# PyLops/pylops-mpi

Measured on AMD Instinct MI355X. Metric: MPIFirstDerivative fp64 matvec+rmatvec pairs/sec, higher is better.
Workload: dtype f64; 1 GPU; MPIFirstDerivative cgls config (BASELINE configs[1]); partition=scatter-axis0, kind=centered, order=3

## Files before the change

include/pam.h:

```cpp
#ifndef PAM_H
#define PAM_H

#include <stdint.h>

#ifdef __cplusplus
extern "C" {
#endif

#define PAM_F64 0
#define PAM_F32 1
#define PAM_C128 2
#define PAM_C64 3

#define PAM_EARG   (-1)
#define PAM_EDTYPE (-2)
#define PAM_EOP    (-3)

int64_t pam_version(void);

int64_t pam_reduce_ws_elems(void);

int pam_fill(void* stream, void* y, int64_t n, double value, int dtype);
int pam_neg(void* stream, void* y, const void* x, int64_t n, int dtype);
int pam_add(void* stream, void* y, const void* a, const void* b, int64_t n,
            int dtype);
int pam_sub(void* stream, void* y, const void* a, const void* b, int64_t n,
            int dtype);
int pam_mul(void* stream, void* y, const void* a, const void* b, int64_t n,
            int dtype);
int pam_scale(void* stream, void* y, const void* x, double alpha, int64_t n,
              int dtype);
int pam_axpy(void* stream, void* y, const void* x, double alpha, int64_t n,
             int dtype);
int pam_xpby(void* stream, void* y, const void* x, double beta, int64_t n,
             int dtype);

int pam_axpy_d(void* stream, void* y, const void* x, const void* alpha,
               double scale, int64_t n, int dtype);
int pam_xpby_d(void* stream, void* y, const void* x, const void* beta,
               double scale, int64_t n, int dtype);
int pam_scalar_alpha(void* stream, void* out, const void* num,
                     const void* den, double damp);
int pam_scalar_div(void* stream, void* out, const void* num, const void* den);

int pam_cmul(void* stream, void* y, const void* a, const void* b, int64_t n,
             int dtype);
int pam_cscale(void* stream, void* y, const void* x, double alpha_re,
               double alpha_im, int64_t n, int dtype);
int pam_conj(void* stream, void* y, const void* x, int64_t n, int dtype);

int pam_thresh(void* stream, void* y, const void* x, int64_t n, int kind,
               double thresh, int dtype);

int pam_dot(void* stream, const void* x, const void* y, int64_t n, void* ws,
            void* out, int dtype);

int pam_cdot(void* stream, const void* x, const void* y, int64_t n,
             int conjx, void* ws, void* out, int dtype);

int pam_norm_local(void* stream, const void* x, int64_t n, int op, double p,
                   void* ws, void* out, int dtype);

#define PAM_GROUP_MAX 4
int pam_group_shrink(void* stream, int mode, int64_t ncomp,
                     void* y0, void* y1, void* y2, void* y3,
                     const void* a0, const void* a1, const void* a2,
                     const void* a3,
                     const void* b0, const void* b1, const void* b2,
                     const void* b3,
                     double beta, int64_t n, double thresh, int dtype);
int pam_group_norm(void* stream, int64_t ncomp,
                   const void* x0, const void* x1, const void* x2,
                   const void* x3,
                   int64_t n, void* ws, void* out, int dtype);

int64_t pam_fd_halo_width(int op);
int pam_fd_apply(void* stream, int op, int edge, const void* x,
                 const void* gf, const void* gb, void* y, int64_t nloc,
                 int64_t m, int64_t row0, int64_t nglob, int64_t rbegin,
                 int64_t rend, double coeff, int dtype);

int pam_nsconv(void* stream, int forward, const void* x, void* y,
               const void* hs, int64_t batch, int64_t d, int64_t m,
               int64_t nf, int64_t hsize, double oh, double dh, int dtype);

int pam_fd_serial(void* stream, int op, int edge, const void* x, void* y,
                  int64_t batch, int64_t d, int64_t m, double coeff,
                  int dtype);

int64_t pam_gemv_ws_elems(int64_t nr, int64_t nc);
int pam_gemv(void* stream, int trans, const void* A, const void* x, void* y,
             int64_t nr, int64_t nc, void* ws, int dtype);

int pam_gemm(void* stream, const void* A, const void* B, void* C, int64_t M,
             int64_t N, int64_t K, int64_t lda, int64_t ldb, int64_t ldc,
             int accumulate, int dtype);
int pam_transpose(void* stream, const void* A, void* At, int64_t nr,
                  int64_t nc, int dtype);

int pam_cgemm_batched(void* stream, const void* A, const void* B, void* C,
                      int64_t batch, int64_t M, int64_t N, int64_t K,
                      int64_t strideA, int64_t strideB, int64_t strideC,
                      int opa, int accumulate, int dtype);

int pam_gemm_batched(void* stream, const void* A, const void* B, void* C,
                     int64_t batch, int64_t M, int64_t N, int64_t K,
                     int64_t strideA, int64_t strideB, int64_t strideC,
                     int opa, int accumulate, int dtype);

int pam_unzip(void* stream, void* dst_real, const void* src_cplx, int64_t n,
              int dtype);
int pam_zip(void* stream, void* dst_cplx, const void* src_real, int64_t n,
            int dtype);

int pam_rfft_strided(void* stream, const void* in_real, void* out_cplx,
                     int64_t nt, int64_t m, int dtype);
int pam_irfft_strided(void* stream, void* in_cplx, void* out_real,
                      int64_t nt, int64_t m, int dtype);

int pam_rfft_contig(void* stream, const void* in_real, void* out_cplx,
                    int64_t nt, int64_t m, int dtype);
int pam_irfft_contig(void* stream, void* in_cplx, void* out_real,
                     int64_t nt, int64_t m, int dtype);

int pam_unzip_t(void* stream, void* dst_real, const void* src_cplx,
                int64_t nt, int64_t m, int dtype);
int pam_zip_t(void* stream, void* dst_cplx, const void* src_real,
              int64_t nt, int64_t m, int dtype);

int pam_gemm_kt(void* stream, const void* At, const void* B, void* C,
                int64_t M, int64_t N, int64_t K, int accumulate,
                int dtype);

int pam_ctranspose(void* stream, const void* A, void* At, int64_t nr,
                   int64_t nc, int conj, int dtype);

#ifdef __cplusplus
}
#endif
#endif
```

pylops_mpi_amd/_ffi.py:

```python
import ctypes
import os

import torch

_LIB_PATH = os.path.join(os.path.dirname(os.path.abspath(__file__)),
                         "libpam.so")
_lib = None
_load_error = None

F64, F32, C128, C64 = 0, 1, 2, 3
_CODES = {torch.float64: F64, torch.float32: F32,
          torch.complex128: C128, torch.complex64: C64}

P, L, I, D = (ctypes.c_void_p, ctypes.c_int64, ctypes.c_int,
              ctypes.c_double)
_SIGS = {
    "pam_version": ([], L),
    "pam_reduce_ws_elems": ([], L),
    "pam_fill": ([P, P, L, D, I], I),
    "pam_neg": ([P, P, P, L, I], I),
    "pam_add": ([P, P, P, P, L, I], I),
    "pam_sub": ([P, P, P, P, L, I], I),
    "pam_mul": ([P, P, P, P, L, I], I),
    "pam_scale": ([P, P, P, D, L, I], I),
    "pam_axpy": ([P, P, P, D, L, I], I),
    "pam_xpby": ([P, P, P, D, L, I], I),
    "pam_axpy_d": ([P, P, P, P, D, L, I], I),
    "pam_xpby_d": ([P, P, P, P, D, L, I], I),
    "pam_scalar_alpha": ([P, P, P, P, D], I),
    "pam_scalar_div": ([P, P, P, P], I),
    "pam_dot": ([P, P, P, L, P, P, I], I),
    "pam_cmul": ([P, P, P, P, L, I], I),
    "pam_cscale": ([P, P, P, D, D, L, I], I),
    "pam_conj": ([P, P, P, L, I], I),
    "pam_thresh": ([P, P, P, L, I, D, I], I),
    "pam_cdot": ([P, P, P, L, I, P, P, I], I),
    "pam_cgemm_batched": ([P, P, P, P, L, L, L, L, L, L, L, I, I, I], I),
    "pam_ctranspose": ([P, P, P, L, L, I, I], I),
    "pam_rfft_strided": ([P, P, P, L, L, I], I),
    "pam_irfft_strided": ([P, P, P, L, L, I], I),
    "pam_rfft_contig": ([P, P, P, L, L, I], I),
    "pam_irfft_contig": ([P, P, P, L, L, I], I),
    "pam_unzip_t": ([P, P, P, L, L, I], I),
    "pam_zip_t": ([P, P, P, L, L, I], I),
    "pam_unzip": ([P, P, P, L, I], I),
    "pam_zip": ([P, P, P, L, I], I),
    "pam_gemm_batched": ([P, P, P, P, L, L, L, L, L, L, L, I, I, I], I),
    "pam_norm_local": ([P, P, L, I, D, P, P, I], I),
    "pam_group_shrink": ([P, I, L, P, P, P, P, P, P, P, P, P, P, P, P, D, L,
                          D, I], I),
    "pam_group_norm": ([P, L, P, P, P, P, L, P, P, I], I),
    "pam_gemv_ws_elems": ([L, L], L),
    "pam_gemv": ([P, I, P, P, P, L, L, P, I], I),
    "pam_gemm": ([P, P, P, P, L, L, L, L, L, L, I, I], I),
    "pam_gemm_kt": ([P, P, P, P, L, L, L, I, I], I),
    "pam_transpose": ([P, P, P, L, L, I], I),
    "pam_fd_halo_width": ([I], L),
    "pam_nsconv": ([P, I, P, P, P, L, L, L, L, L, D, D, I], I),
    "pam_fd_serial": ([P, I, I, P, P, L, L, L, D, I], I),
    "pam_fd_apply": ([P, I, I, P, P, P, P, L, L, L, L, L, L, D, I], I),
}


def lib():
    global _lib, _load_error
    if _lib is not None:
        return _lib
    if _load_error is not None:
        raise _load_error
    try:
        so = ctypes.CDLL(_LIB_PATH)
        for name, (argtypes, restype) in _SIGS.items():
            fn = getattr(so, name)
            fn.argtypes = argtypes
            fn.restype = restype
        ver = so.pam_version()
        if ver != 1:
            raise RuntimeError(f"pam ABI version mismatch: {ver}")
    except OSError as e:
        _load_error = ImportError(
            f"pam HIP extension not found/loadable at {_LIB_PATH} "
            f"(build it with __graft_entry__.build()): {e}")
        raise _load_error
    _lib = so
    return so


def available() -> bool:
    try:
        lib()
        return True
    except ImportError:
        return False


def checked(rc: int, what: str) -> None:
    if rc != 0:
        raise RuntimeError(f"pam: {what} failed with code {rc}")


def dtype_code(torch_dtype) -> int:
    try:
        return _CODES[torch_dtype]
    except KeyError:
        raise TypeError(f"pam: unsupported dtype {torch_dtype}") from None
```

pylops_mpi_amd/csrc/pam.hip:

```cpp

#include <hip/hip_runtime.h>
#include <math.h>
#include <stdint.h>
#include <stdlib.h>
#include <utility>

#include "../../include/pam.h"
#include "fd_defs.h"

#define PAM_ABI_VERSION 1
#define BLK 256
#define NPARTIAL 1024

extern "C" int64_t pam_version(void) { return PAM_ABI_VERSION; }
extern "C" int64_t pam_reduce_ws_elems(void) { return NPARTIAL; }

static inline int check(hipError_t e) { return (int)e; }

static inline int64_t grid_1d(int64_t work) {
  static int64_t cap = [] {
    const char* e = getenv("PAM_EW_CAP");
    return (int64_t)(e ? atoll(e) : 0x7FFFFFFF);
  }();
  int64_t g = (work + BLK - 1) / BLK;
// ... 957 lines not shown
static int group_norm_nc(void* stream, int64_t ncomp, const void* const* x,
                         int64_t n, void* ws, void* out) {
  switch (ncomp) {
    case 1: return group_norm_launch<T, CPLX, 1>(stream, x, n, ws, out);
    case 2: return group_norm_launch<T, CPLX, 2>(stream, x, n, ws, out);
    case 3: return group_norm_launch<T, CPLX, 3>(stream, x, n, ws, out);
    default: return group_norm_launch<T, CPLX, 4>(stream, x, n, ws, out);
  }
}

extern "C" int pam_group_norm(void* stream, int64_t ncomp, const void* x0,
                              const void* x1, const void* x2, const void* x3,
                              int64_t n, void* ws, void* out, int dtype) {
  const void* const x[PAM_GROUP_MAX] = {x0, x1, x2, x3};
  if (ncomp < 1 || ncomp > PAM_GROUP_MAX) return PAM_EARG;
  for (int64_t c = 0; c < ncomp; ++c)
    if (!x[c]) return PAM_EARG;
  if (n < 0 || !ws || !out) return PAM_EARG;
  if (dtype < PAM_F64 || dtype > PAM_C64) return PAM_EDTYPE;
  if (n == 0)
    return check(hipMemsetAsync(out, 0, sizeof(double), (hipStream_t)stream));
  switch (dtype) {
    case PAM_F64: return group_norm_nc<double, false>(stream, ncomp, x, n, ws, out);
    case PAM_F32: return group_norm_nc<float, false>(stream, ncomp, x, n, ws, out);
    case PAM_C128: return group_norm_nc<double, true>(stream, ncomp, x, n, ws, out);
    default: return group_norm_nc<float, true>(stream, ncomp, x, n, ws, out);
  }
}

#define GEMV_CHUNKS 64

extern "C" int64_t pam_gemv_ws_elems(int64_t nr, int64_t nc) {
  (void)nr;
  return GEMV_CHUNKS * nc;
}

template <typename T, int V>
__global__ void __launch_bounds__(BLK) gemv_n_kernel(
    const T* __restrict__ A, const T* __restrict__ x, T* __restrict__ y,
    int64_t nr, int64_t nc) {
  const int64_t wave = ((int64_t)blockIdx.x * (BLK / 64))
                       + (threadIdx.x >> 6);
  const int lane = threadIdx.x & 63;
  const int64_t nwaves = (int64_t)gridDim.x * (BLK / 64);
  const int64_t ncv = nc / V;
  for (int64_t r = wave; r < nr; r += nwaves) {
    const T* __restrict__ row = A + r * nc;
    double acc = 0.0;
    for (int64_t cv = lane; cv < ncv; cv += 64) {
      T a[V], b[V];
      loadv<T, V>(row + cv * V, a);
      loadv<T, V>(x + cv * V, b);
#pragma unroll
      for (int k = 0; k < V; ++k) acc += (double)a[k] * (double)b[k];
    }
    for (int64_t c = ncv * V + lane; c < nc; c += 64)
      acc += (double)row[c] * (double)x[c];
#pragma unroll
    for (int off = 32; off > 0; off >>= 1) acc += __shfl_down(acc, off, 64);
    if (lane == 0) y[r] = (T)acc;
  }
}

template <typename T, int V>
__global__ void __launch_bounds__(BLK) gemv_t_stage1(
    const T* __restrict__ A, const T* __restrict__ x,
    double* __restrict__ partials, int64_t nr, int64_t nc) {
  const int64_t c0 = ((int64_t)blockIdx.x * BLK + threadIdx.x) * V;
  const int chunk = blockIdx.y;
  const int64_t r0 = (nr * chunk) / GEMV_CHUNKS;
  const int64_t r1 = (nr * (chunk + 1)) / GEMV_CHUNKS;
  if (c0 >= nc) return;
  double acc[V] = {};
  for (int64_t r = r0; r < r1; ++r) {
    T v[V];
    loadv<T, V>(A + r * nc + c0, v);
#pragma unroll
    for (int j = 0; j < V; ++j)
      acc[j] += (double)v[j] * (double)x[r];
  }
#pragma unroll
  for (int j = 0; j < V; ++j)
    partials[(int64_t)chunk * nc + c0 + j] = acc[j];
}

template <typename T>
__global__ void __launch_bounds__(BLK) gemv_t_stage2(
    const double* __restrict__ partials, T* __restrict__ y, int64_t nc) {
  const int64_t c = (int64_t)blockIdx.x * BLK + threadIdx.x;
  if (c >= nc) return;
  double acc = 0.0;
  for (int ch = 0; ch < GEMV_CHUNKS; ++ch)
    acc += partials[(int64_t)ch * nc + c];
  y[c] = (T)acc;
}

template <typename T>
static int gemv_launch(void* stream, int trans, const void* A, const void* x,
                       void* y, int64_t nr, int64_t nc, void* ws) {
  if (nr <= 0 || nc <= 0 || !A || !x || !y) return PAM_EARG;
  hipStream_t s = (hipStream_t)stream;
  if (!trans) {
    constexpr int V = VecW<T>::value;
    const bool vec_ok = (nc % V == 0) && ((uintptr_t)A % 16 == 0) &&
                        ((uintptr_t)x % 16 == 0);
    int64_t nb = (nr + (BLK / 64) - 1) / (BLK / 64);
    if (nb > 4096) nb = 4096;
    if (vec_ok)
      hipLaunchKernelGGL((gemv_n_kernel<T, V>), dim3((uint32_t)nb), dim3(BLK),
                         0, s, (const T*)A, (const T*)x, (T*)y, nr, nc);
    else
      hipLaunchKernelGGL((gemv_n_kernel<T, 1>), dim3((uint32_t)nb), dim3(BLK),
                         0, s, (const T*)A, (const T*)x, (T*)y, nr, nc);
    return check(hipGetLastError());
  }
  if (!ws) return PAM_EARG;
  constexpr int V = VecW<T>::value;
  const bool vec_ok = (nc % V == 0) && ((uintptr_t)A % 16 == 0);
  const int64_t ncl = vec_ok ? nc / V : nc;
  dim3 g1((uint32_t)((ncl + BLK - 1) / BLK), GEMV_CHUNKS);
  if (vec_ok)
    hipLaunchKernelGGL((gemv_t_stage1<T, V>), g1, dim3(BLK), 0, s,
                       (const T*)A, (const T*)x, (double*)ws, nr, nc);
  else
    hipLaunchKernelGGL((gemv_t_stage1<T, 1>), g1, dim3(BLK), 0, s,
                       (const T*)A, (const T*)x, (double*)ws, nr, nc);
  hipError_t e = hipGetLastError();
  if (e != hipSuccess) return (int)e;
  hipLaunchKernelGGL((gemv_t_stage2<T>),
                     dim3((uint32_t)((nc + BLK - 1) / BLK)), dim3(BLK), 0, s,
                     (const double*)ws, (T*)y, nc);
  return check(hipGetLastError());
}

extern "C" int pam_gemv(void* stream, int trans, const void* A, const void* x,
                        void* y, int64_t nr, int64_t nc, void* ws, int dtype) {
  if (dtype == PAM_F64)
    return gemv_launch<double>(stream, trans, A, x, y, nr, nc, ws);
  if (dtype == PAM_F32)
    return gemv_launch<float>(stream, trans, A, x, y, nr, nc, ws);
  return PAM_EDTYPE;
}


extern "C" int64_t pam_fd_halo_width(int op) {
  switch (op) {
    case 0: case 1: case 2: case 3: case 4: case 5: return 1;
    case 6: case 7: case 8: case 9: case 10: case 11: case 12: case 13:
      return 2;
    default: return PAM_EOP;
  }
}

template <typename T, int OP, int V, bool NTS = false, bool RSWAP = false>
__global__ void __launch_bounds__(BLK) fd_kernel(Rows<T> R, T* __restrict__ y,
                                                 int64_t row0, int64_t N, T c,
                                                 int edge, int64_t rbegin,
                                                 int64_t rend) {
  const int64_t brow = RSWAP ? blockIdx.x : blockIdx.y;
  const int64_t grows = RSWAP ? gridDim.x : gridDim.y;
  const int64_t bcol = RSWAP ? blockIdx.y : blockIdx.x;
  const int64_t gcols = RSWAP ? gridDim.y : gridDim.x;
  const int64_t m = R.m, mv = m / V;
  const int64_t cstride = (int64_t)gcols * blockDim.x;
  for (int64_t i = rbegin + brow; i < rend; i += grows) {
    const int64_t g = row0 + i;
    T* __restrict__ yrow = y + i * m;
    for (int64_t jv = (int64_t)bcol * blockDim.x + threadIdx.x; jv < mv;
         jv += cstride) {
      const int64_t j = jv * V;
      T acc[V];
#pragma unroll
      for (int k = 0; k < V; ++k) acc[k] = (T)0;
#pragma unroll
      for (int t = 0; t < FDDef<OP>::NT; ++t) {
        const Term tm = FDDef<OP>::TERMS[t];
        if (g >= tm.lo && g <= N - 1 - tm.hi) {
          T v[V];
          loadv<T, V>(R.row(i + tm.off) + j, v);
#pragma unroll
          for (int k = 0; k < V; ++k) acc[k] += (T)tm.coeff * v[k];
        }
      }
      if (edge) fd_edge<T, OP, V>(R, i, j, g, N, acc);
#pragma unroll
      for (int k = 0; k < V; ++k) acc[k] *= c;
      storev_p<T, V, NTS>(yrow + j, acc);
    }
    if constexpr (V > 1) {
      for (int64_t j = mv * V + (int64_t)bcol * blockDim.x + threadIdx.x;
           j < m; j += cstride) {
        T acc[1] = {(T)0};
#pragma unroll
        for (int t = 0; t < FDDef<OP>::NT; ++t) {
          const Term tm = FDDef<OP>::TERMS[t];
          if (g >= tm.lo && g <= N - 1 - tm.hi)
            acc[0] += (T)tm.coeff * R.row(i + tm.off)[j];
        }
        if (edge) fd_edge<T, OP, 1>(R, i, j, g, N, acc);
        const T o = acc[0] * c;
        if constexpr (NTS)
          __builtin_nontemporal_store(o, yrow + j);
        else
          yrow[j] = o;
      }
    }
  }
}


template <typename T, int OP, int V, int W, int t>
__device__ __forceinline__ void roll_term(const T (&win)[2 * W + 1][V],
                                          T (&acc)[V], int64_t g,
                                          int64_t N) {
  constexpr Term tm = FDDef<OP>::TERMS[t];
  if (g >= tm.lo && g <= N - 1 - tm.hi) {
#pragma unroll
    for (int k = 0; k < V; ++k)
      acc[k] += (T)tm.coeff * win[tm.off + W][k];
  }
}

template <typename T, int OP, int V, int W, int... Ts>
__device__ __forceinline__ void roll_terms(const T (&win)[2 * W + 1][V],
                                           T (&acc)[V], int64_t g,
                                           int64_t N,
                                           std::integer_sequence<int, Ts...>) {
  (roll_term<T, OP, V, W, Ts>(win, acc, g, N), ...);
}

template <typename T, int OP, int V, int CV, bool NTS = false,
          bool NTL = false>
__global__ void __launch_bounds__(BLK) fd_roll_kernel(
    Rows<T> R, T* __restrict__ y, int64_t row0, int64_t N, T c, int edge,
    int64_t rbegin, int64_t rend) {
  constexpr int W = FDDef<OP>::W;
  constexpr int NROLL = 2 * W + 1;
  const int64_t m = R.m, mv = m / V;
  const int64_t base = (int64_t)blockIdx.x * blockDim.x * CV + threadIdx.x;
  const int64_t nr = rend - rbegin;
  const int64_t c0 = rbegin + (nr * blockIdx.y) / gridDim.y;
  const int64_t c1 = rbegin + (nr * (blockIdx.y + 1)) / gridDim.y;
  if (c1 <= c0 || base >= mv) return;
  const int64_t lo = R.gf ? -(int64_t)R.w : 0;
  const int64_t hi = R.nloc - 1 + (R.gb ? R.w : 0);
  auto clamp_row = [&](int64_t i) {
    return i < lo ? lo : (i > hi ? hi : i);
  };
  int64_t js[CV];
  bool vq[CV];
#pragma unroll
  for (int q = 0; q < CV; ++q) {
    const int64_t jq = base + (int64_t)q * blockDim.x;
    vq[q] = jq < mv;
    js[q] = (vq[q] ? jq : mv - 1) * V;
  }
  T buf[CV][NROLL][V];
#pragma unroll
  for (int q = 0; q < CV; ++q)
#pragma unroll
    for (int k = 0; k < NROLL; ++k)
      if constexpr (NTL) loadv_nt<T, V>(R.row(clamp_row(c0 - W + k)) + js[q], buf[q][k]);
      else loadv<T, V>(R.row(clamp_row(c0 - W + k)) + js[q], buf[q][k]);
  for (int64_t i = c0; i < c1; ++i) {
    const int64_t g = row0 + i;
    T nxt[CV][V];
    const int64_t rn = clamp_row(i + 1 + W);
#pragma unroll
    for (int q = 0; q < CV; ++q)
      if constexpr (NTL) loadv_nt<T, V>(R.row(rn) + js[q], nxt[q]);
      else loadv<T, V>(R.row(rn) + js[q], nxt[q]);
#pragma unroll
    for (int q = 0; q < CV; ++q) {
      T acc[V];
#pragma unroll
      for (int k = 0; k < V; ++k) acc[k] = (T)0;
      roll_terms<T, OP, V, W>(
          buf[q], acc, g, N,
          std::make_integer_sequence<int, FDDef<OP>::NT>{});
      if (edge) fd_edge<T, OP, V>(R, i, js[q], g, N, acc);
#pragma unroll
      for (int k = 0; k < V; ++k) acc[k] *= c;
      if (vq[q]) storev_p<T, V, NTS>(y + i * m + js[q], acc);
#pragma unroll
      for (int k = 0; k < NROLL - 1; ++k)
#pragma unroll
        for (int v = 0; v < V; ++v) buf[q][k][v] = buf[q][k + 1][v];
#pragma unroll
      for (int v = 0; v < V; ++v) buf[q][NROLL - 1][v] = nxt[q][v];
    }
  }
}

template <int... Us, typename F>
__device__ __forceinline__ void fd_static_for(
    std::integer_sequence<int, Us...>, F&& f) {
  (f(std::integral_constant<int, Us>{}), ...);
}

template <typename T, int OP, int V, int W, int ROT, int t>
__device__ __forceinline__ void roll2_term(const T (&win)[2 * W + 1][V],
                                           T (&acc)[V], int64_t g,
                                           int64_t N) {
  constexpr Term tm = FDDef<OP>::TERMS[t];
  constexpr int NR = 2 * W + 1;
  constexpr int slot = ((tm.off + W + ROT) % NR + NR) % NR;
  if (g >= tm.lo && g <= N - 1 - tm.hi) {
#pragma unroll
    for (int k = 0; k < V; ++k)
      acc[k] += (T)tm.coeff * win[slot][k];
  }
}

template <typename T, int OP, int V, int W, int ROT, int... Ts>
__device__ __forceinline__ void roll2_terms(
    const T (&win)[2 * W + 1][V], T (&acc)[V], int64_t g, int64_t N,
    std::integer_sequence<int, Ts...>) {
  (roll2_term<T, OP, V, W, ROT, Ts>(win, acc, g, N), ...);
}

template <typename T, int OP, int V, int CV, bool NTS = false>
__global__ void __launch_bounds__(BLK) fd_roll2_kernel(
    Rows<T> R, T* __restrict__ y, int64_t row0, int64_t N, T c, int edge,
    int64_t rbegin, int64_t rend) {
  constexpr int W = FDDef<OP>::W;
  constexpr int NROLL = 2 * W + 1;
  const int64_t m = R.m, mv = m / V;
  const int64_t base = (int64_t)blockIdx.x * blockDim.x * CV + threadIdx.x;
  const int64_t nr = rend - rbegin;
  const int64_t c0 = rbegin + (nr * blockIdx.y) / gridDim.y;
  const int64_t c1 = rbegin + (nr * (blockIdx.y + 1)) / gridDim.y;
  if (c1 <= c0 || base >= mv) return;
  const int64_t lo = R.gf ? -(int64_t)R.w : 0;
  const int64_t hi = R.nloc - 1 + (R.gb ? R.w : 0);
  auto clamp_row = [&](int64_t i) {
    return i < lo ? lo : (i > hi ? hi : i);
  };
  int64_t js[CV];
  bool vq[CV];
#pragma unroll
  for (int q = 0; q < CV; ++q) {
    const int64_t jq = base + (int64_t)q * blockDim.x;
    vq[q] = jq < mv;
    js[q] = (vq[q] ? jq : mv - 1) * V;
  }
  T buf[CV][NROLL][V];
#pragma unroll
  for (int q = 0; q < CV; ++q)
#pragma unroll
    for (int k = 0; k < NROLL; ++k)
      loadv<T, V>(R.row(clamp_row(c0 - W + k)) + js[q], buf[q][k]);
  int64_t i = c0;
  auto step = [&](auto rotc) {
    constexpr int ROT = decltype(rotc)::value;
    constexpr int oldest = ROT % NROLL;
    const int64_t rn = clamp_row(i + W + 1);
    T nxt[CV][V];
#pragma unroll
    for (int q = 0; q < CV; ++q)
      loadv<T, V>(R.row(rn) + js[q], nxt[q]);
    const int64_t g = row0 + i;
#pragma unroll
    for (int q = 0; q < CV; ++q) {
      T acc[V];
#pragma unroll
      for (int k = 0; k < V; ++k) acc[k] = (T)0;
      roll2_terms<T, OP, V, W, ROT>(
          buf[q], acc, g, N,
          std::make_integer_sequence<int, FDDef<OP>::NT>{});
      if (edge) fd_edge<T, OP, V>(R, i, js[q], g, N, acc);
#pragma unroll
      for (int k = 0; k < V; ++k) acc[k] *= c;
      if (vq[q]) storev_p<T, V, NTS>(y + i * m + js[q], acc);
#pragma unroll
      for (int v = 0; v < V; ++v) buf[q][oldest][v] = nxt[q][v];
    }
    ++i;
  };
  while (i + NROLL <= c1)
    fd_static_for(std::make_integer_sequence<int, NROLL>{},
                  [&](auto rc) { step(rc); });
  fd_static_for(std::make_integer_sequence<int, NROLL>{}, [&](auto rc) {
    if (i < c1) step(rc);
  });
}

static int fd_vec_override() {
  static int v = [] {
    const char* e = getenv("PAM_FD_VEC");
    return e ? atoi(e) : 0;
  }();
  return v;
}

static int fd_nt_override() {
  static int v = [] {
    const char* e = getenv("PAM_FD_NT");
    return e ? atoi(e) : 0;
  }();
  return v;
}

template <typename T, int OP>
static int fd_launch(void* stream, int edge, const void* x, const void* gf,
                     const void* gb, void* y, int64_t nloc, int64_t m,
                     int64_t row0, int64_t nglob, int64_t rbegin,
                     int64_t rend, double coeff) {
  if (nloc < 0 || m <= 0 || rbegin < 0 || rend > nloc) return PAM_EARG;
  const int64_t nrows = rend - rbegin;
  if (nloc == 0 || nrows <= 0) return 0;
  Rows<T> R{(const T*)x, (const T*)gf, (const T*)gb, nloc, m, FDDef<OP>::W};
  const bool align16 = ((uintptr_t)x % 16 == 0) && ((uintptr_t)y % 16 == 0) &&
                       (gf == nullptr || (uintptr_t)gf % 16 == 0) &&
                       (gb == nullptr || (uintptr_t)gb % 16 == 0);
  int V = 1;
  if (align16) {
    if (sizeof(T) == 8)
      V = (m % 2 == 0) ? 2 : 1;
    else
      V = (m % 4 == 0) ? 4 : 1;
    const int ov = fd_vec_override();
    if ((ov == 1 || ov == 2 || ov == 4) && m % ov == 0) V = ov;
  }
  const int64_t mv = m / V;
  static int gycap = [] {
    const char* e = getenv("PAM_FD_GY");
    return e ? atoi(e) : 65535;
  }();
  static int totcap = [] {
    const char* e = getenv("PAM_FD_CAP");
    return e ? atoi(e) : 262144;
  }();
  int gy = (int)(nrows < gycap ? nrows : gycap);
  if (gy < 1) gy = 1;
  int64_t gx64 = (mv + BLK - 1) / BLK;
  int64_t cap = totcap / gy;
  if (cap < 1) cap = 1;
  if (gx64 > cap) gx64 = cap;
  dim3 grid((uint32_t)gx64, (uint32_t)gy);
  hipStream_t s = (hipStream_t)stream;
  static int rollov = [] {
    const char* e = getenv("PAM_FD_ROLL");
    return e ? atoi(e) : 0;
  }();
  static int64_t longrow = [] {
    const char* e = getenv("PAM_FD_LONGROW");
    return (int64_t)(e ? atoll(e) : (4 << 20));
  }();
  const int64_t rowbytes = m * (int64_t)sizeof(T);
  const bool roll_auto =
      rollov == 0 && V > 1 &&
      (rowbytes > longrow ||
       (rowbytes * 8 >= longrow * 5 && (nrows % 1024) != 0));
  static int rolltgt = [] {
    const char* e = getenv("PAM_FD_ROLL_TGT");
    return e ? atoi(e) : 2048;
  }();
  if ((rollov > 0 && V > 1) || roll_auto) {
    if (roll_auto && fd_vec_override() == 0 && m % 4 == 0 && align16)
      V = 4;
    static int cvov = [] {
      const char* e = getenv("PAM_FD_ROLL_CV");
      return e ? atoi(e) : 8;
    }();
    const int CV = (cvov == 2 || cvov == 4) ? cvov : 8;
    const int64_t mv2 = m / V;
    int64_t gx = (mv2 + (int64_t)BLK * CV - 1) / ((int64_t)BLK * CV);
    int64_t gyr = rolltgt / (gx ? gx : 1);
    const int64_t minchunk = 16;
    int64_t maxgy = (nrows + minchunk - 1) / minchunk;
    if (gyr > maxgy) gyr = maxgy;
    if (gyr < 1) gyr = 1;
    if (gyr > 65535) gyr = 65535;
    dim3 gridr((uint32_t)gx, (uint32_t)gyr);
    const bool rnt = fd_nt_override() != 0;
    static int ntlov = [] {
      const char* e = getenv("PAM_FD_NTL");
      return e ? atoi(e) : 0;
    }();
    const bool rntl = ntlov != 0;
#define ROLL_LAUNCH(KER, VV, CC)                                              \
  do {                                                                        \
    if (rnt)                                                                  \
      hipLaunchKernelGGL((KER<T, OP, VV, CC, true>), gridr, dim3(BLK), 0, s,  \
                         R, (T*)y, row0, nglob, (T)coeff, edge, rbegin,       \
                         rend);                                               \
    else                                                                      \
      hipLaunchKernelGGL((KER<T, OP, VV, CC, false>), gridr, dim3(BLK), 0, s, \
                         R, (T*)y, row0, nglob, (T)coeff, edge, rbegin,       \
                         rend);                                               \
  } while (0)
#define ROLL_LAUNCH1(VV, CC)                                                  \
  do {                                                                        \
    if (rntl)                                                                 \
      hipLaunchKernelGGL((fd_roll_kernel<T, OP, VV, CC, false, true>),        \
                         gridr, dim3(BLK), 0, s, R, (T*)y, row0, nglob,       \
                         (T)coeff, edge, rbegin, rend);                       \
    else                                                                      \
      ROLL_LAUNCH(fd_roll_kernel, VV, CC);                                    \
  } while (0)
    if (rollov == 2) {
      if (V == 4 && CV == 2) ROLL_LAUNCH(fd_roll2_kernel, 4, 2);
      else if (V == 4 && CV == 8) ROLL_LAUNCH(fd_roll2_kernel, 4, 8);
      else if (V == 4) ROLL_LAUNCH(fd_roll2_kernel, 4, 4);
      else if (CV == 2) ROLL_LAUNCH(fd_roll2_kernel, 2, 2);
      else if (CV == 8) ROLL_LAUNCH(fd_roll2_kernel, 2, 8);
      else ROLL_LAUNCH(fd_roll2_kernel, 2, 4);
    } else {
      if (V == 4 && CV == 2) ROLL_LAUNCH1(4, 2);
      else if (V == 4 && CV == 8) ROLL_LAUNCH1(4, 8);
      else if (V == 4) ROLL_LAUNCH1(4, 4);
      else if (CV == 2) ROLL_LAUNCH1(2, 2);
      else if (CV == 8) ROLL_LAUNCH1(2, 8);
      else ROLL_LAUNCH1(2, 4);
    }
#undef ROLL_LAUNCH1
#undef ROLL_LAUNCH
    return check(hipGetLastError());
  }
  static int rswap = [] {
    const char* e = getenv("PAM_FD_RSWAP");
    return e ? atoi(e) : 0;
  }();
  if (rswap) {
    dim3 grid_s((uint32_t)gy, (uint32_t)gx64);
    if (V == 4)
      hipLaunchKernelGGL((fd_kernel<T, OP, 4, false, true>), grid_s,
                         dim3(BLK), 0, s, R, (T*)y, row0, nglob, (T)coeff,
                         edge, rbegin, rend);
    else if (V == 2 && sizeof(T) == 8)
      hipLaunchKernelGGL((fd_kernel<T, OP, 2, false, true>), grid_s,
                         dim3(BLK), 0, s, R, (T*)y, row0, nglob, (T)coeff,
                         edge, rbegin, rend);
    else
      hipLaunchKernelGGL((fd_kernel<T, OP, 1, false, true>), grid_s,
                         dim3(BLK), 0, s, R, (T*)y, row0, nglob, (T)coeff,
                         edge, rbegin, rend);
    return check(hipGetLastError());
  }
  const bool nt = fd_nt_override() != 0;
  if (nt) {
    if (V == 4)
      hipLaunchKernelGGL((fd_kernel<T, OP, 4, true>), grid, dim3(BLK), 0, s,
                         R, (T*)y, row0, nglob, (T)coeff, edge, rbegin, rend);
    else if (V == 2 && sizeof(T) == 8)
      hipLaunchKernelGGL((fd_kernel<T, OP, 2, true>), grid, dim3(BLK), 0, s,
                         R, (T*)y, row0, nglob, (T)coeff, edge, rbegin, rend);
    else
      hipLaunchKernelGGL((fd_kernel<T, OP, 1, true>), grid, dim3(BLK), 0, s,
                         R, (T*)y, row0, nglob, (T)coeff, edge, rbegin, rend);
  } else if (V == 4)
    hipLaunchKernelGGL((fd_kernel<T, OP, 4>), grid, dim3(BLK), 0, s, R, (T*)y,
                       row0, nglob, (T)coeff, edge, rbegin, rend);
  else if (V == 2 && sizeof(T) == 8)
    hipLaunchKernelGGL((fd_kernel<T, OP, 2>), grid, dim3(BLK), 0, s, R, (T*)y,
                       row0, nglob, (T)coeff, edge, rbegin, rend);
  else
    hipLaunchKernelGGL((fd_kernel<T, OP, 1>), grid, dim3(BLK), 0, s, R, (T*)y,
                       row0, nglob, (T)coeff, edge, rbegin, rend);
  return check(hipGetLastError());
}

extern "C" int pam_fd_apply(void* stream, int op, int edge, const void* x,
                            const void* gf, const void* gb, void* y,
                            int64_t nloc, int64_t m, int64_t row0,
                            int64_t nglob, int64_t rbegin, int64_t rend,
                            double coeff, int dtype) {
#define FD_CASE(T)                                                            \
  switch (op) {                                                               \
    case 0: return fd_launch<T, 0>(stream, edge, x, gf, gb, y, nloc, m, row0, nglob, rbegin, rend, coeff); \
    case 1: return fd_launch<T, 1>(stream, edge, x, gf, gb, y, nloc, m, row0, nglob, rbegin, rend, coeff); \
    case 2: return fd_launch<T, 2>(stream, edge, x, gf, gb, y, nloc, m, row0, nglob, rbegin, rend, coeff); \
    case 3: return fd_launch<T, 3>(stream, edge, x, gf, gb, y, nloc, m, row0, nglob, rbegin, rend, coeff); \
    case 4: return fd_launch<T, 4>(stream, edge, x, gf, gb, y, nloc, m, row0, nglob, rbegin, rend, coeff); \
    case 5: return fd_launch<T, 5>(stream, edge, x, gf, gb, y, nloc, m, row0, nglob, rbegin, rend, coeff); \
    case 6: return fd_launch<T, 6>(stream, edge, x, gf, gb, y, nloc, m, row0, nglob, rbegin, rend, coeff); \
    case 7: return fd_launch<T, 7>(stream, edge, x, gf, gb, y, nloc, m, row0, nglob, rbegin, rend, coeff); \
    case 8: return fd_launch<T, 8>(stream, edge, x, gf, gb, y, nloc, m, row0, nglob, rbegin, rend, coeff); \
    case 9: return fd_launch<T, 9>(stream, edge, x, gf, gb, y, nloc, m, row0, nglob, rbegin, rend, coeff); \
    case 10: return fd_launch<T, 10>(stream, edge, x, gf, gb, y, nloc, m, row0, nglob, rbegin, rend, coeff); \
    case 11: return fd_launch<T, 11>(stream, edge, x, gf, gb, y, nloc, m, row0, nglob, rbegin, rend, coeff); \
    case 12: return fd_launch<T, 12>(stream, edge, x, gf, gb, y, nloc, m, row0, nglob, rbegin, rend, coeff); \
    case 13: return fd_launch<T, 13>(stream, edge, x, gf, gb, y, nloc, m, row0, nglob, rbegin, rend, coeff); \
    default: return PAM_EOP;                                                  \
  }
  if (dtype == PAM_F64) { FD_CASE(double) }
  if (dtype == PAM_F32) { FD_CASE(float) }
#undef FD_CASE
  return PAM_EDTYPE;
}
```

pylops_mpi_amd/kernels.py:

```python
from functools import lru_cache

import torch
from torch import Tensor

from . import _ffi
from ._ffi import dtype_code as _code

_REAL_OF = {torch.complex128: torch.float64, torch.complex64: torch.float32}
_F64 = torch.float64


_AS_REAL = {torch.complex128: (2, _ffi.F64), torch.complex64: (2, _ffi.F32)}


def _real_code(t):
    return _AS_REAL.get(t.dtype) or (1, _code(t.dtype))


def _typed(name, dtype, *ts):
    for t in ts:
        if t.dtype != dtype:
            raise TypeError(f"pam: {name}: expected {dtype}, got {t.dtype}")


# ... 196 lines not shown
    if idx not in _reduce_scratch:
        nws, dev = int(_ffi.lib().pam_reduce_ws_elems()), ins[0].device
        _reduce_scratch[idx] = (torch.empty(2 * nws, dtype=_F64, device=dev),
                                torch.empty(2, dtype=_F64, device=dev))
    ws, cached = _reduce_scratch[idx]
    out = cached[:nout] if out is None else out
    ptrs = [t.data_ptr() for t in ins] + [None] * (slots - len(ins))
    _launch(idx, name, (*pre, *ptrs, n, *extras, ws.data_ptr(),
                        out.data_ptr(), dt))
    return out


def dot(x, y, out=None):
    return _reduce("pam_dot", (x, y), (), out, 1)


def cdot(x, y, conjx: bool, out=None):
    return _reduce("pam_cdot", (x, y), (1 if conjx else 0,), out, 2)


def norm_local(x, op: int, p: float, out=None):
    return _reduce("pam_norm_local", (x,), (int(op), float(p)), out, 1)


def group_norm(xs, out=None):
    nc, _, _ = _group("pam_group_norm", xs)
    return _reduce("pam_group_norm", tuple(xs), (), out, 1, pre=(nc,),
                   slots=_GROUP_MAX)


_gemv_scratch = {}


def gemv(y, A, x, trans: bool):
    name = "pam_gemv"
    nr, nc = A.shape
    _typed(name, A.dtype, x, y)
    _sized(name, nr if trans else nc, x)
    _sized(name, nc if trans else nr, y)
    _dst(name, y)
    A, x = A.contiguous(), x.contiguous()
    idx = require_device(y, A, x)
    need = int(_ffi.lib().pam_gemv_ws_elems(nr, nc))
    ws = _gemv_scratch.get(idx)
    if ws is None or ws.numel() < need:
        ws = _gemv_scratch[idx] = torch.empty(need, dtype=_F64,
                                              device=y.device)
    _launch(idx, name, (1 if trans else 0, A.data_ptr(), x.data_ptr(),
                        y.data_ptr(), nr, nc, ws.data_ptr(), _code(A.dtype)))


def gemm(C, A, B, accumulate: bool = False):
    if C.is_complex():
        return gemm_batched(C[None], A[None], B[None], False, accumulate)
    (M, K), N = A.shape, B.shape[-1]
    _typed("pam_gemm", C.dtype, A, B)
    _shaped("pam_gemm", (K, N), B)
    _shaped("pam_gemm", (M, N), _dst("pam_gemm", C))
    _run("pam_gemm", A.contiguous(), B.contiguous(), C, M, N, K, K, N, N,
         1 if accumulate else 0, _code(C.dtype))


def gemm_batched(C, A, B, opa: bool = False, accumulate: bool = False):
    name = "pam_cgemm_batched" if C.is_complex() else "pam_gemm_batched"
    batch, d1, d2 = A.shape
    (K, M), N = ((d1, d2) if opa else (d2, d1)), B.shape[-1]
    _typed(name, C.dtype, A, B)
    _shaped(name, (batch, K, N), B)
    _shaped(name, (batch, M, N), _dst(name, C))
    _run(name, A.contiguous(), B.contiguous(), C, batch, M, N, K, M * K,
         K * N, M * N, 1 if opa else 0, 1 if accumulate else 0,
         _code(C.dtype))


def transpose(At, A, conj: bool = False):
    name = "pam_ctranspose" if A.is_complex() else "pam_transpose"
    nr, nc = A.shape
    _typed(name, A.dtype, At)
    _shaped(name, (nc, nr), _dst(name, At))
    flag = (1 if conj else 0,) if A.is_complex() else ()
    _run(name, A.contiguous(), At, nr, nc, *flag, _code(A.dtype))


def _cplx_real(name, c, r):
    if not c.is_complex():
        raise TypeError(f"pam: {name}: expected complex, got {c.dtype}")
    _typed(name, _REAL_OF[c.dtype], r)


def _zip(name, dst, src, cplx, real, transposed):
    name += "_t" if transposed else ""
    _cplx_real(name, cplx, real)
    if transposed:
        dims = nt, m = cplx.shape
        _shaped(name, (m, nt), real)
    else:
        dims = (cplx.numel(),)
        _sized(name, *dims, real)
    _run(name, _dst(name, dst), src.contiguous(), *dims, _code(cplx.dtype))


def unzip(dst_real, src_cplx, transposed=False):
    _zip("pam_unzip", dst_real, src_cplx, src_cplx, dst_real, transposed)


def zip(dst_cplx, src_real, transposed=False):
    _zip("pam_zip", dst_cplx, src_real, dst_cplx, src_real, transposed)


def _rfft(name, dst, src, cplx, real, contig):
    name += "_contig" if contig else "_strided"
    _cplx_real(name, cplx, real)
    m, nt = real.shape if contig else real.shape[::-1]
    _shaped(name, (m, nt // 2 + 1) if contig else (nt // 2 + 1, m), cplx)
    _run(name, src.contiguous(), _dst(name, dst), nt, m, _code(real.dtype))


def rfft(out_cplx, in_real, contig: bool):
    _rfft("pam_rfft", out_cplx, in_real, out_cplx, in_real, contig)


def irfft(out_real, in_cplx, contig: bool):
    _rfft("pam_irfft", out_real, in_cplx, in_cplx, out_real, contig)


@lru_cache(maxsize=None)
def fd_halo_width(op: int) -> int:
    return int(_ffi.lib().pam_fd_halo_width(int(op)))


def fd_apply(y, x, gf, gb, op: int, edge: bool, row0: int, nglob: int,
             rbegin: int, rend: int, coeff: float):
    name = "pam_fd_apply"
    k, dt = _real_code(y)
    nloc, m = x.shape
    halo = (fd_halo_width(op), m)
    for t, shape in ((x, y.shape), (gf, halo), (gb, halo)):
        if t is not None and (t.dtype != y.dtype or t.shape != shape):
            _typed(name, y.dtype, t)
            _shaped(name, shape, t)
    if not 0 <= rbegin <= rend <= nloc:
        raise ValueError(f"pam: {name}: rows [{rbegin}, {rend}) outside "
                         f"the {nloc}-row block")
    x, gf, gb = (t if t is None else t.contiguous() for t in (x, gf, gb))
    idx = require_device(*[t for t in (_dst(name, y), x, gf, gb)
                           if t is not None])
    _launch(idx, name, (
        int(op), 1 if edge else 0, x.data_ptr(),
        None if gf is None else gf.data_ptr(),
        None if gb is None else gb.data_ptr(), y.data_ptr(), nloc, k * m,
        int(row0), int(nglob), int(rbegin), int(rend), float(coeff), dt))


def fd_serial(y, x, op: int, edge: bool, coeff: float):
    _typed("pam_fd_serial", y.dtype, x)
    k, dt = _real_code(y)
    batch, d, m = x.shape
    _shaped("pam_fd_serial", (batch, d, m), _dst("pam_fd_serial", y))
    _run("pam_fd_serial", int(op), 1 if edge else 0, x.contiguous(), y,
         batch, d, k * m, float(coeff), dt)


def nsconv(y, x, hs, forward: bool, oh: float, dh: float):
    _typed("pam_nsconv", y.dtype, x, hs)
    (batch, d, m), (nf, hsize) = x.shape, hs.shape
    _shaped("pam_nsconv", (batch, d, m), _dst("pam_nsconv", y))
    _run("pam_nsconv", 1 if forward else 0, x.contiguous(), y,
         hs.contiguous(), batch, d, m, nf, hsize, float(oh), float(dh),
         _code(y.dtype))
```

Measured before the change: 336.1 pairs/s.

## Add register-banded FD kernel and unrolled interior fast path for row stencil

```diff
diff --git a/include/pam.h b/include/pam.h
--- a/include/pam.h
+++ b/include/pam.h
@@ -79,6 +79,8 @@
                  const void* gf, const void* gb, void* y, int64_t nloc,
                  int64_t m, int64_t row0, int64_t nglob, int64_t rbegin,
                  int64_t rend, double coeff, int dtype);
+int pam_fd_variant(int dtype, int64_t m, int64_t nrows, int aligned16);
+int64_t pam_fd_band_rows(void);
 
 int pam_nsconv(void* stream, int forward, const void* x, void* y,
                const void* hs, int64_t batch, int64_t d, int64_t m,
diff --git a/pylops_mpi_amd/_ffi.py b/pylops_mpi_amd/_ffi.py
--- a/pylops_mpi_amd/_ffi.py
+++ b/pylops_mpi_amd/_ffi.py
@@ -59,6 +59,8 @@
     "pam_nsconv": ([P, I, P, P, P, L, L, L, L, L, D, D, I], I),
     "pam_fd_serial": ([P, I, I, P, P, L, L, L, D, I], I),
     "pam_fd_apply": ([P, I, I, P, P, P, P, L, L, L, L, L, L, D, I], I),
+    "pam_fd_variant": ([I, L, L, I], I),
+    "pam_fd_band_rows": ([], L),
 }
 
 
diff --git a/pylops_mpi_amd/csrc/pam.hip b/pylops_mpi_amd/csrc/pam.hip
--- a/pylops_mpi_amd/csrc/pam.hip
+++ b/pylops_mpi_amd/csrc/pam.hip
@@ -1133,28 +1133,82 @@
   }
 }
 
-template <typename T, int OP, int V, bool NTS = false, bool RSWAP = false>
+template <int OP>
+constexpr int fd_margin() {
+  int mg = 3;
+  for (int t = 0; t < FDDef<OP>::NT; ++t) {
+    if (FDDef<OP>::TERMS[t].lo > mg) mg = FDDef<OP>::TERMS[t].lo;
+    if (FDDef<OP>::TERMS[t].hi > mg) mg = FDDef<OP>::TERMS[t].hi;
+  }
+  return mg;
+}
+
+template <typename T, int OP, int V, bool NTS = false, int U = 1>
 __global__ void __launch_bounds__(BLK) fd_kernel(Rows<T> R, T* __restrict__ y,
                                                  int64_t row0, int64_t N, T c,
                                                  int edge, int64_t rbegin,
                                                  int64_t rend) {
-  const int64_t brow = RSWAP ? blockIdx.x : blockIdx.y;
-  const int64_t grows = RSWAP ? gridDim.x : gridDim.y;
-  const int64_t bcol = RSWAP ? blockIdx.y : blockIdx.x;
-  const int64_t gcols = RSWAP ? gridDim.y : gridDim.x;
+  constexpr int W = FDDef<OP>::W, MG = fd_margin<OP>();
+  constexpr int NTm = FDDef<OP>::NT;
+  const int64_t bcol = blockIdx.x;
   const int64_t m = R.m, mv = m / V;
-  const int64_t cstride = (int64_t)gcols * blockDim.x;
-  for (int64_t i = rbegin + brow; i < rend; i += grows) {
+  const int64_t cstride = (int64_t)gridDim.x * blockDim.x;
+  for (int64_t i = rbegin + blockIdx.y; i < rend; i += gridDim.y) {
     const int64_t g = row0 + i;
     T* __restrict__ yrow = y + i * m;
-    for (int64_t jv = (int64_t)bcol * blockDim.x + threadIdx.x; jv < mv;
-         jv += cstride) {
+    int64_t jv = (int64_t)bcol * blockDim.x + threadIdx.x;
+    if (i >= W && i + W < R.nloc && g >= MG && g <= N - 1 - MG) {
+      const T* __restrict__ xrow = R.x + i * m;
+      if constexpr (U > 1) {
+        for (; jv + (U - 1) * cstride < mv; jv += U * cstride) {
+          T v[U][NTm][V];
+#pragma unroll
+          for (int u = 0; u < U; ++u)
+#pragma unroll
+            for (int t = 0; t < NTm; ++t)
+              loadv<T, V>(xrow + FDDef<OP>::TERMS[t].off * m +
+                              (jv + u * cstride) * V, v[u][t]);
+#pragma unroll
+          for (int u = 0; u < U; ++u) {
+            T acc[V];
+#pragma unroll
+            for (int k = 0; k < V; ++k) acc[k] = (T)0;
+#pragma unroll
+            for (int t = 0; t < NTm; ++t)
+#pragma unroll
+              for (int k = 0; k < V; ++k)
+                acc[k] += (T)FDDef<OP>::TERMS[t].coeff * v[u][t][k];
+#pragma unroll
+            for (int k = 0; k < V; ++k) acc[k] *= c;
+            storev_p<T, V, NTS>(yrow + (jv + u * cstride) * V, acc);
+          }
+        }
+      }
+      for (; jv < mv; jv += cstride) {
+        const int64_t j = jv * V;
+        T acc[V];
+#pragma unroll
+        for (int k = 0; k < V; ++k) acc[k] = (T)0;
+#pragma unroll
+        for (int t = 0; t < NTm; ++t) {
+          T v[V];
+          loadv<T, V>(xrow + FDDef<OP>::TERMS[t].off * m + j, v);
+#pragma unroll
+          for (int k = 0; k < V; ++k)
+            acc[k] += (T)FDDef<OP>::TERMS[t].coeff * v[k];
+        }
+#pragma unroll
+        for (int k = 0; k < V; ++k) acc[k] *= c;
+        storev_p<T, V, NTS>(yrow + j, acc);
+      }
+    }
+    for (; jv < mv; jv += cstride) {
       const int64_t j = jv * V;
       T acc[V];
 #pragma unroll
       for (int k = 0; k < V; ++k) acc[k] = (T)0;
 #pragma unroll
-      for (int t = 0; t < FDDef<OP>::NT; ++t) {
+      for (int t = 0; t < NTm; ++t) {
         const Term tm = FDDef<OP>::TERMS[t];
         if (g >= tm.lo && g <= N - 1 - tm.hi) {
           T v[V];
@@ -1189,6 +1243,88 @@
   }
 }
 
+#ifndef PAM_FD_BAND_RT
+#define PAM_FD_BAND_RT 4
+#endif
+
+template <typename T, int OP, int V, int RT, int r, int t>
+__device__ __forceinline__ void band_term(
+    const T (&in)[RT + 2 * FDDef<OP>::W][V], T (&acc)[V]) {
+  constexpr Term tm = FDDef<OP>::TERMS[t];
+#pragma unroll
+  for (int k = 0; k < V; ++k)
+    acc[k] += (T)tm.coeff * in[r + tm.off + FDDef<OP>::W][k];
+}
+
+template <typename T, int OP, int V, int RT, int r, int... Ts>
+__device__ __forceinline__ void band_terms(
+    const T (&in)[RT + 2 * FDDef<OP>::W][V], T (&acc)[V],
+    std::integer_sequence<int, Ts...>) {
+  (band_term<T, OP, V, RT, r, Ts>(in, acc), ...);
+}
+
+template <int... Us, typename F>
+__device__ __forceinline__ void fd_static_for(
+    std::integer_sequence<int, Us...>, F&& f) {
+  (f(std::integral_constant<int, Us>{}), ...);
+}
+
+template <typename T, int OP, int V, int RT>
+__global__ void __launch_bounds__(BLK) fd_band_kernel(
+    Rows<T> R, T* __restrict__ y, int64_t row0, int64_t N, T c, int edge,
+    int64_t rbegin, int64_t rend, uint32_t ncb) {
+  constexpr int W = FDDef<OP>::W;
+  constexpr int MG = fd_margin<OP>();
+  const uint32_t band = blockIdx.x / ncb, cb = blockIdx.x - band * ncb;
+  const int64_t m = R.m;
+  const int64_t jv = (int64_t)cb * BLK + threadIdx.x;
+  if (jv >= m / V) return;
+  const int64_t j = jv * V;
+  const int64_t i0 = rbegin + (int64_t)band * RT;
+  const int64_t g0 = row0 + i0;
+  const bool interior = i0 - W >= 0 && i0 + RT - 1 + W < R.nloc &&
+                        i0 + RT <= rend && g0 >= MG &&
+                        g0 + RT - 1 <= N - 1 - MG;
+  if (interior) {
+    const T* __restrict__ p = R.x + (i0 - W) * m + j;
+    T in[RT + 2 * W][V];
+#pragma unroll
+    for (int k = 0; k < RT + 2 * W; ++k) loadv<T, V>(p + k * m, in[k]);
+    T* __restrict__ q = y + i0 * m + j;
+    fd_static_for(std::make_integer_sequence<int, RT>{}, [&](auto rc) {
+      constexpr int r = decltype(rc)::value;
+      T acc[V];
+#pragma unroll
+      for (int k = 0; k < V; ++k) acc[k] = (T)0;
+      band_terms<T, OP, V, RT, r>(
+          in, acc, std::make_integer_sequence<int, FDDef<OP>::NT>{});
+#pragma unroll
+      for (int k = 0; k < V; ++k) acc[k] *= c;
+      storev<T, V>(q + r * m, acc);
+    });
+    return;
+  }
+  for (int64_t i = i0; i < i0 + RT && i < rend; ++i) {
+    const int64_t g = row0 + i;
+    T acc[V];
+#pragma unroll
+    for (int k = 0; k < V; ++k) acc[k] = (T)0;
+#pragma unroll
+    for (int t = 0; t < FDDef<OP>::NT; ++t) {
+      const Term tm = FDDef<OP>::TERMS[t];
+      if (g >= tm.lo && g <= N - 1 - tm.hi) {
+        T v[V];
+        loadv<T, V>(R.row(i + tm.off) + j, v);
+#pragma unroll
+        for (int k = 0; k < V; ++k) acc[k] += (T)tm.coeff * v[k];
+      }
+    }
+    if (edge) fd_edge<T, OP, V>(R, i, j, g, N, acc);
+#pragma unroll
+    for (int k = 0; k < V; ++k) acc[k] *= c;
+    storev<T, V>(y + i * m + j, acc);
+  }
+}
 
 template <typename T, int OP, int V, int W, int t>
 __device__ __forceinline__ void roll_term(const T (&win)[2 * W + 1][V],
@@ -1273,99 +1409,6 @@
   }
 }
 
-template <int... Us, typename F>
-__device__ __forceinline__ void fd_static_for(
-    std::integer_sequence<int, Us...>, F&& f) {
-  (f(std::integral_constant<int, Us>{}), ...);
-}
-
-template <typename T, int OP, int V, int W, int ROT, int t>
-__device__ __forceinline__ void roll2_term(const T (&win)[2 * W + 1][V],
-                                           T (&acc)[V], int64_t g,
-                                           int64_t N) {
-  constexpr Term tm = FDDef<OP>::TERMS[t];
-  constexpr int NR = 2 * W + 1;
-  constexpr int slot = ((tm.off + W + ROT) % NR + NR) % NR;
-  if (g >= tm.lo && g <= N - 1 - tm.hi) {
-#pragma unroll
-    for (int k = 0; k < V; ++k)
-      acc[k] += (T)tm.coeff * win[slot][k];
-  }
-}
-
-template <typename T, int OP, int V, int W, int ROT, int... Ts>
-__device__ __forceinline__ void roll2_terms(
-    const T (&win)[2 * W + 1][V], T (&acc)[V], int64_t g, int64_t N,
-    std::integer_sequence<int, Ts...>) {
-  (roll2_term<T, OP, V, W, ROT, Ts>(win, acc, g, N), ...);
-}
-
-template <typename T, int OP, int V, int CV, bool NTS = false>
-__global__ void __launch_bounds__(BLK) fd_roll2_kernel(
-    Rows<T> R, T* __restrict__ y, int64_t row0, int64_t N, T c, int edge,
-    int64_t rbegin, int64_t rend) {
-  constexpr int W = FDDef<OP>::W;
-  constexpr int NROLL = 2 * W + 1;
-  const int64_t m = R.m, mv = m / V;
-  const int64_t base = (int64_t)blockIdx.x * blockDim.x * CV + threadIdx.x;
-  const int64_t nr = rend - rbegin;
-  const int64_t c0 = rbegin + (nr * blockIdx.y) / gridDim.y;
-  const int64_t c1 = rbegin + (nr * (blockIdx.y + 1)) / gridDim.y;
-  if (c1 <= c0 || base >= mv) return;
-  const int64_t lo = R.gf ? -(int64_t)R.w : 0;
-  const int64_t hi = R.nloc - 1 + (R.gb ? R.w : 0);
-  auto clamp_row = [&](int64_t i) {
-    return i < lo ? lo : (i > hi ? hi : i);
-  };
-  int64_t js[CV];
-  bool vq[CV];
-#pragma unroll
-  for (int q = 0; q < CV; ++q) {
-    const int64_t jq = base + (int64_t)q * blockDim.x;
-    vq[q] = jq < mv;
-    js[q] = (vq[q] ? jq : mv - 1) * V;
-  }
-  T buf[CV][NROLL][V];
-#pragma unroll
-  for (int q = 0; q < CV; ++q)
-#pragma unroll
-    for (int k = 0; k < NROLL; ++k)
-      loadv<T, V>(R.row(clamp_row(c0 - W + k)) + js[q], buf[q][k]);
-  int64_t i = c0;
-  auto step = [&](auto rotc) {
-    constexpr int ROT = decltype(rotc)::value;
-    constexpr int oldest = ROT % NROLL;
-    const int64_t rn = clamp_row(i + W + 1);
-    T nxt[CV][V];
-#pragma unroll
-    for (int q = 0; q < CV; ++q)
-      loadv<T, V>(R.row(rn) + js[q], nxt[q]);
-    const int64_t g = row0 + i;
-#pragma unroll
-    for (int q = 0; q < CV; ++q) {
-      T acc[V];
-#pragma unroll
-      for (int k = 0; k < V; ++k) acc[k] = (T)0;
-      roll2_terms<T, OP, V, W, ROT>(
-          buf[q], acc, g, N,
-          std::make_integer_sequence<int, FDDef<OP>::NT>{});
-      if (edge) fd_edge<T, OP, V>(R, i, js[q], g, N, acc);
-#pragma unroll
-      for (int k = 0; k < V; ++k) acc[k] *= c;
-      if (vq[q]) storev_p<T, V, NTS>(y + i * m + js[q], acc);
-#pragma unroll
-      for (int v = 0; v < V; ++v) buf[q][oldest][v] = nxt[q][v];
-    }
-    ++i;
-  };
-  while (i + NROLL <= c1)
-    fd_static_for(std::make_integer_sequence<int, NROLL>{},
-                  [&](auto rc) { step(rc); });
-  fd_static_for(std::make_integer_sequence<int, NROLL>{}, [&](auto rc) {
-    if (i < c1) step(rc);
-  });
-}
-
 static int fd_vec_override() {
   static int v = [] {
     const char* e = getenv("PAM_FD_VEC");
@@ -1381,6 +1424,64 @@
   }();
   return v;
 }
+
+static int fd_roll_override() {
+  static int v = [] {
+    const char* e = getenv("PAM_FD_ROLL");
+    return e ? atoi(e) : 0;
+  }();
+  return v;
+}
+
+static int64_t fd_longrow() {
+  static int64_t v = [] {
+    const char* e = getenv("PAM_FD_LONGROW");
+    return (int64_t)(e ? atoll(e) : (4 << 20));
+  }();
+  return v;
+}
+
+static int fd_vec_width(int tsize, int64_t m, bool align16) {
+  if (!align16) return 1;
+  const int vw = 16 / tsize;
+  int V = (m % vw == 0) ? vw : 1;
+  const int ov = fd_vec_override();
+  if ((ov == 1 || ov == 2 || ov == 4) && m % ov == 0) V = ov;
+  return V;
+}
+
+static bool fd_band_auto(int64_t rowbytes, int64_t nrows, int64_t longrow) {
+  return rowbytes <= longrow && rowbytes * 8 >= longrow * 5 &&
+         (nrows % 1024) != 0 && nrows >= 4 * PAM_FD_BAND_RT;
+}
+
+static int fd_variant(int tsize, int64_t m, int64_t nrows, bool align16) {
+  const int V = fd_vec_width(tsize, m, align16);
+  const bool band_ok = V > 1 && V == 16 / tsize;
+  const char* e = getenv("PAM_FD_BAND");
+  const int bandov = e ? atoi(e) : 0;
+  if (bandov > 0 && band_ok && nrows >= 1) return 2;
+  const int rollov = fd_roll_override();
+  const int64_t rowbytes = m * (int64_t)tsize;
+  const int64_t longrow = fd_longrow();
+  const bool roll_shape =
+      rowbytes > longrow ||
+      (rowbytes * 8 >= longrow * 5 && (nrows % 1024) != 0);
+  if (bandov == 0 && rollov == 0 && band_ok &&
+      fd_band_auto(rowbytes, nrows, longrow))
+    return 2;
+  if (V > 1 && (rollov > 0 || (rollov == 0 && roll_shape))) return 1;
+  return 0;
+}
+
+extern "C" int pam_fd_variant(int dtype, int64_t m, int64_t nrows,
+                              int aligned16) {
+  if (dtype != PAM_F64 && dtype != PAM_F32) return PAM_EDTYPE;
+  if (m <= 0 || nrows < 0) return PAM_EARG;
+  return fd_variant(dtype == PAM_F64 ? 8 : 4, m, nrows, aligned16 != 0);
+}
+
+extern "C" int64_t pam_fd_band_rows(void) { return PAM_FD_BAND_RT; }
 
 template <typename T, int OP>
 static int fd_launch(void* stream, int edge, const void* x, const void* gf,
@@ -1394,14 +1495,19 @@
   const bool align16 = ((uintptr_t)x % 16 == 0) && ((uintptr_t)y % 16 == 0) &&
                        (gf == nullptr || (uintptr_t)gf % 16 == 0) &&
                        (gb == nullptr || (uintptr_t)gb % 16 == 0);
-  int V = 1;
-  if (align16) {
-    if (sizeof(T) == 8)
-      V = (m % 2 == 0) ? 2 : 1;
-    else
-      V = (m % 4 == 0) ? 4 : 1;
-    const int ov = fd_vec_override();
-    if ((ov == 1 || ov == 2 || ov == 4) && m % ov == 0) V = ov;
+  int V = fd_vec_width((int)sizeof(T), m, align16);
+  const int variant = fd_variant((int)sizeof(T), m, nrows, align16);
+  hipStream_t s = (hipStream_t)stream;
+  if (variant == 2) {
+    constexpr int BV = VecW<T>::value, RT = PAM_FD_BAND_RT;
+    const int64_t ncb = (m / BV + BLK - 1) / BLK;
+    const int64_t nbands = (nrows + RT - 1) / RT;
+    if (ncb * nbands > 0x7fffffffLL) return PAM_EARG;
+    hipLaunchKernelGGL((fd_band_kernel<T, OP, BV, RT>),
+                       dim3((uint32_t)(ncb * nbands)), dim3(BLK), 0, s, R,
+                       (T*)y, row0, nglob, (T)coeff, edge, rbegin, rend,
+                       (uint32_t)ncb);
+    return check(hipGetLastError());
   }
   const int64_t mv = m / V;
   static int gycap = [] {
@@ -1419,25 +1525,13 @@
   if (cap < 1) cap = 1;
   if (gx64 > cap) gx64 = cap;
   dim3 grid((uint32_t)gx64, (uint32_t)gy);
-  hipStream_t s = (hipStream_t)stream;
-  static int rollov = [] {
-    const char* e = getenv("PAM_FD_ROLL");
-    return e ? atoi(e) : 0;
-  }();
-  static int64_t longrow = [] {
-    const char* e = getenv("PAM_FD_LONGROW");
-    return (int64_t)(e ? atoll(e) : (4 << 20));
-  }();
-  const int64_t rowbytes = m * (int64_t)sizeof(T);
-  const bool roll_auto =
-      rollov == 0 && V > 1 &&
-      (rowbytes > longrow ||
-       (rowbytes * 8 >= longrow * 5 && (nrows % 1024) != 0));
+  const int rollov = fd_roll_override();
+  const bool roll_auto = rollov == 0 && variant == 1;
   static int rolltgt = [] {
     const char* e = getenv("PAM_FD_ROLL_TGT");
     return e ? atoi(e) : 2048;
   }();
-  if ((rollov > 0 && V > 1) || roll_auto) {
+  if (variant == 1) {
     if (roll_auto && fd_vec_override() == 0 && m % 4 == 0 && align16)
       V = 4;
     static int cvov = [] {
@@ -1480,43 +1574,14 @@
     else                                                                      \
       ROLL_LAUNCH(fd_roll_kernel, VV, CC);                                    \
   } while (0)
-    if (rollov == 2) {
-      if (V == 4 && CV == 2) ROLL_LAUNCH(fd_roll2_kernel, 4, 2);
-      else if (V == 4 && CV == 8) ROLL_LAUNCH(fd_roll2_kernel, 4, 8);
-      else if (V == 4) ROLL_LAUNCH(fd_roll2_kernel, 4, 4);
-      else if (CV == 2) ROLL_LAUNCH(fd_roll2_kernel, 2, 2);
-      else if (CV == 8) ROLL_LAUNCH(fd_roll2_kernel, 2, 8);
-      else ROLL_LAUNCH(fd_roll2_kernel, 2, 4);
-    } else {
-      if (V == 4 && CV == 2) ROLL_LAUNCH1(4, 2);
-      else if (V == 4 && CV == 8) ROLL_LAUNCH1(4, 8);
-      else if (V == 4) ROLL_LAUNCH1(4, 4);
-      else if (CV == 2) ROLL_LAUNCH1(2, 2);
-      else if (CV == 8) ROLL_LAUNCH1(2, 8);
-      else ROLL_LAUNCH1(2, 4);
-    }
+    if (V == 4 && CV == 2) ROLL_LAUNCH1(4, 2);
+    else if (V == 4 && CV == 8) ROLL_LAUNCH1(4, 8);
+    else if (V == 4) ROLL_LAUNCH1(4, 4);
+    else if (CV == 2) ROLL_LAUNCH1(2, 2);
+    else if (CV == 8) ROLL_LAUNCH1(2, 8);
+    else ROLL_LAUNCH1(2, 4);
 #undef ROLL_LAUNCH1
 #undef ROLL_LAUNCH
-    return check(hipGetLastError());
-  }
-  static int rswap = [] {
-    const char* e = getenv("PAM_FD_RSWAP");
-    return e ? atoi(e) : 0;
-  }();
-  if (rswap) {
-    dim3 grid_s((uint32_t)gy, (uint32_t)gx64);
-    if (V == 4)
-      hipLaunchKernelGGL((fd_kernel<T, OP, 4, false, true>), grid_s,
-                         dim3(BLK), 0, s, R, (T*)y, row0, nglob, (T)coeff,
-                         edge, rbegin, rend);
-    else if (V == 2 && sizeof(T) == 8)
-      hipLaunchKernelGGL((fd_kernel<T, OP, 2, false, true>), grid_s,
-                         dim3(BLK), 0, s, R, (T*)y, row0, nglob, (T)coeff,
-                         edge, rbegin, rend);
-    else
-      hipLaunchKernelGGL((fd_kernel<T, OP, 1, false, true>), grid_s,
-                         dim3(BLK), 0, s, R, (T*)y, row0, nglob, (T)coeff,
-                         edge, rbegin, rend);
     return check(hipGetLastError());
   }
   const bool nt = fd_nt_override() != 0;
@@ -1530,7 +1595,11 @@
     else
       hipLaunchKernelGGL((fd_kernel<T, OP, 1, true>), grid, dim3(BLK), 0, s,
                          R, (T*)y, row0, nglob, (T)coeff, edge, rbegin, rend);
-  } else if (V == 4)
+  } else if (V == VecW<T>::value && (mv + BLK - 1) / BLK >= 4 * gx64)
+    hipLaunchKernelGGL((fd_kernel<T, OP, VecW<T>::value, false, 4>), grid,
+                       dim3(BLK), 0, s, R, (T*)y, row0, nglob, (T)coeff, edge,
+                       rbegin, rend);
+  else if (V == 4)
     hipLaunchKernelGGL((fd_kernel<T, OP, 4>), grid, dim3(BLK), 0, s, R, (T*)y,
                        row0, nglob, (T)coeff, edge, rbegin, rend);
   else if (V == 2 && sizeof(T) == 8)
diff --git a/pylops_mpi_amd/kernels.py b/pylops_mpi_amd/kernels.py
--- a/pylops_mpi_amd/kernels.py
+++ b/pylops_mpi_amd/kernels.py
@@ -372,6 +372,26 @@
         int(row0), int(nglob), int(rbegin), int(rend), float(coeff), dt))
 
 
+FD_ROW, FD_ROLL, FD_BAND = 0, 1, 2
+
+
+def fd_band_rows() -> int:
+    return int(_ffi.lib().pam_fd_band_rows())
+
+
+def fd_variant(y, x, gf, gb, rbegin: int, rend: int) -> int:
+    k, dt = _real_code(y)
+    x, gf, gb = (t if t is None else t.contiguous() for t in (x, gf, gb))
+    aligned = all(t.data_ptr() % 16 == 0 for t in (y, x, gf, gb)
+                  if t is not None)
+    v = int(_ffi.lib().pam_fd_variant(dt, k * x.shape[1],
+                                      int(rend) - int(rbegin),
+                                      1 if aligned else 0))
+    if v < 0:
+        _ffi.checked(v, "pam_fd_variant")
+    return v
+
+
 def fd_serial(y, x, op: int, edge: bool, coeff: float):
     _typed("pam_fd_serial", y.dtype, x)
     k, dt = _real_code(y)
```

New measurement: 349.0 pairs/s, median of 6. 3.8% higher.
